# wienkers/marEx

Hardware: AMD Instinct MI355X
Metric: Mcells*timesteps/s, shifting_baseline + hobday_extreme p95 (validation+anomaly+thresholds+mask) (higher is better)
Workload: dtype f32

## Files before the change

### marex_amd/csrc/build.py

```python
import os
import subprocess
import sys
from concurrent.futures import ThreadPoolExecutor

HERE = os.path.dirname(os.path.abspath(__file__))
ROOT = os.path.dirname(os.path.dirname(HERE))
UNITS = ["marex_context", "marex_synth", "marex_shifting", "marex_thresholds", "marex_mask", "marex_anomalies",
         "marex_quantiles", "marex_morphology", "marex_objects", "marex_mesh_objects", "marex_merge", "marex_blosc", "marex_tails", "marex_zstd"]
SRC = [os.path.join(HERE, u + ".hip") for u in UNITS]
HEADERS = [os.path.join(HERE, "marex_common.hip.h"), os.path.join(HERE, "marex_tails.hip.h"), os.path.join(ROOT, "include", "marex_hip.h")]
OUT = os.path.join(HERE, "libmarex_hip.so")
FLAGS = [
    "--offload-arch=gfx950", "-O3", "-std=c++17", "-fPIC",
    "-ffp-contract=off",
    "-fno-fast-math", "-Wall", "-Wno-unused-result", "-Wno-unused-function",
    "-I", os.path.join(ROOT, "include"),
]


def _obj(src: str) -> str:
    return src[:-4] + ".o"


def _stale(target: str, deps) -> bool:
    if not os.path.exists(target):
        return True
    t = os.path.getmtime(target)
    return any(os.path.getmtime(d) > t for d in deps)


def needs_build() -> bool:
    return _stale(OUT, SRC + HEADERS + [os.path.abspath(__file__)])


def build(force: bool = False, verbose: bool = True) -> str:
    hipcc = os.environ.get("HIPCC", "/opt/rocm/bin/hipcc")
    extra = os.environ.get("MAREX_HIPCC_FLAGS", "").split()
    todo = [s for s in SRC if force or extra or _stale(_obj(s), [s] + HEADERS + [os.path.abspath(__file__)])]

    def compile_one(src):
        cmd = [hipcc, *FLAGS, *extra, "-c", src, "-o", _obj(src)]
        if verbose:
            print(" ".join(cmd), flush=True)
# ... 16 lines not shown
```

### marex_amd/csrc/marex_common.hip.h

```cpp
#pragma once
#include <hip/hip_runtime.h>

#include <cmath>
#include <type_traits>
#include <cstdarg>
#include <cstdio>
#include <cstring>
#include <map>
#include <string>
#include <vector>

#include "marex_hip.h"

#define NDOY MAREX_NDOY

struct TimedLaunch {
    int kid;
    hipEvent_t a, b;
};

struct marex_ctx {
    int device = 0;
    hipStream_t stream = nullptr;
    std::string err;
    bool timing = false;
    std::vector<TimedLaunch> pending;
    double total_ms[MAREX_K_COUNT] = {0};
    int64_t launches[MAREX_K_COUNT] = {0};
    int* shift_info = nullptr;
    int* shift_plan = nullptr;
    size_t shift_plan_years = 0;
    int* shift_lplan = nullptr;
    size_t shift_lplan_years = 0;
    unsigned char* thr_scratch = nullptr;
    size_t thr_scratch_bytes = 0;
    unsigned char* detrend_scratch = nullptr;
    size_t detrend_scratch_bytes = 0;
    unsigned char* morph_scratch = nullptr;
    size_t morph_scratch_bytes = 0;
    int n_cu = 0;
    std::map<std::string, int> opts;
    long long* row_off = nullptr;
    size_t row_off_bytes = 0;
    long long* row_off_mask = nullptr;
    size_t row_off_mask_bytes = 0;
    unsigned long long* dbg_counters = nullptr;
};

#define MAREX_DBG_COUNTERS 8

static inline int ctx_opt(marex_ctx* ctx, const char* name, int dflt) {
    auto it = ctx->opts.find(name);
    return it == ctx->opts.end() ? dflt : it->second;
}

#ifdef MAREX_ABLATION
#define MAREX_ABLATE_OPT(ctx, name) ctx_opt(ctx, name, 0)
#else
#define MAREX_ABLATE_OPT(ctx, name) 0
#endif

static inline unsigned long long* ctx_debug_counters(marex_ctx* ctx) {
    if (!ctx->dbg_counters) {
        if (hipMalloc((void**)&ctx->dbg_counters, MAREX_DBG_COUNTERS * sizeof(unsigned long long)) != hipSuccess) return nullptr;
        (void)hipMemsetAsync(ctx->dbg_counters, 0, MAREX_DBG_COUNTERS * sizeof(unsigned long long), ctx->stream);
    }
    return ctx->dbg_counters;
}
// ... 145 lines not shown
```

### marex_amd/csrc/marex_context.hip

```cpp
#include "marex_common.hip.h"

extern "C" int marex_abi_version(void) { return MAREX_ABI_VERSION; }

extern "C" int marex_workspace_bytes(const marex_workspace_cfg* cfg, size_t* bytes) {
    if (!cfg || !bytes || cfg->T <= 0 || cfg->T_out <= 0 || cfg->T_out > cfg->T || cfg->C <= 0) return -1;
    const size_t C = (size_t)cfg->C, To = (size_t)cfg->T_out;
    for (int i = 0; i < MAREX_WS_COUNT; ++i) bytes[i] = 0;
    bytes[MAREX_WS_ANOMALY] = To * C * sizeof(float);
    bytes[MAREX_WS_EXTREME] = To * C;
    bytes[MAREX_WS_THRESHOLDS] = (size_t)MAREX_NDOY * C * sizeof(float);
    if (cfg->list_rows > 0) {
        const int nper = marex_tail_lists(cfg->max_bucket, cfg->list_rows);
        if (nper < 1) return -1;
        const size_t nch = cfg->list_rows <= 16 ? 2 : 4;
        bytes[MAREX_WS_LISTS] = (size_t)MAREX_NDOY * (size_t)nper * nch * C * 16;
        bytes[MAREX_WS_AUX] = (size_t)MAREX_NDOY * C * sizeof(uint32_t);
    } else {
        bytes[MAREX_WS_BINS] = ((C + 15) / 16) * To * 16 * sizeof(uint16_t);
    }
    bytes[MAREX_WS_PER_CELL] = C * (sizeof(uint8_t) + sizeof(int32_t));
    bytes[MAREX_WS_TOTAL] = bytes[MAREX_WS_ANOMALY] + bytes[MAREX_WS_EXTREME] + 2 * bytes[MAREX_WS_THRESHOLDS] + bytes[MAREX_WS_LISTS] +
                            bytes[MAREX_WS_AUX] + bytes[MAREX_WS_BINS] + bytes[MAREX_WS_PER_CELL];
    return 0;
}
// ... 21 lines not shown
extern "C" int marex_set_option(marex_ctx* ctx, const char* name, int value) {
    if (!ctx || !name || !*name) return -1;
    ctx->opts[name] = value;
    return 0;
}

extern "C" int marex_clear_option(marex_ctx* ctx, const char* name) {
    if (!ctx) return -1;
    if (!name)
        ctx->opts.clear();
    else
        ctx->opts.erase(name);
    return 0;
}

extern "C" int marex_debug_counters(marex_ctx* ctx, uint64_t* out, int reset) {
    if (!ctx || !out) return -1;
    HIP_TRY(ctx, hipSetDevice(ctx->device));
    unsigned long long* d = ctx_debug_counters(ctx);
    if (!d) return fail(ctx, -2, "marex_debug_counters: allocation failed");
    HIP_TRY(ctx, hipStreamSynchronize(ctx->stream));
    HIP_TRY(ctx, hipMemcpy(out, d, MAREX_DBG_COUNTERS * sizeof(unsigned long long), hipMemcpyDeviceToHost));
    if (reset) HIP_TRY(ctx, hipMemsetAsync(d, 0, MAREX_DBG_COUNTERS * sizeof(unsigned long long), ctx->stream));
    return 0;
}

extern "C" int marex_destroy(marex_ctx* ctx) {
    if (!ctx) return -1;
    drain_timers(ctx);
    if (ctx->shift_info) (void)hipFree(ctx->shift_info);
    if (ctx->shift_plan) (void)hipFree(ctx->shift_plan);
    if (ctx->shift_lplan) (void)hipFree(ctx->shift_lplan);
    if (ctx->thr_scratch) (void)hipFree(ctx->thr_scratch);
    if (ctx->detrend_scratch) (void)hipFree(ctx->detrend_scratch);
    if (ctx->morph_scratch) (void)hipFree(ctx->morph_scratch);
    if (ctx->dbg_counters) (void)hipFree(ctx->dbg_counters);
    if (ctx->row_off) (void)hipFree(ctx->row_off);
    if (ctx->row_off_mask) (void)hipFree(ctx->row_off_mask);
    delete ctx;
    return 0;
}

extern "C" const char* marex_last_error(marex_ctx* ctx) { return ctx ? ctx->err.c_str() : "null context"; }

extern "C" int marex_set_stream(marex_ctx* ctx, void* s) {
    if (!ctx) return -1;
    ctx->stream = (hipStream_t)s;
    return 0;
}

extern "C" int marex_sync(marex_ctx* ctx) {
    if (!ctx) return -1;
    HIP_TRY(ctx, hipSetDevice(ctx->device));
    HIP_TRY(ctx, hipStreamSynchronize(ctx->stream));
    drain_timers(ctx);
    return 0;
}

extern "C" int marex_timing_enable(marex_ctx* ctx, int on) {
    if (!ctx) return -1;
    ctx->timing = on != 0;
    return 0;
}

extern "C" int marex_timing_reset(marex_ctx* ctx) {
    if (!ctx) return -1;
// ... 14 lines not shown
```

### marex_amd/csrc/marex_tails.hip

```cpp
#include "marex_common.hip.h"
#include "marex_tails.hip.h"

typedef __amdgpu_buffer_rsrc_t tl_rsrc_t;
__device__ __forceinline__ tl_rsrc_t tl_make_rsrc(const void* base) {
    return __builtin_amdgcn_make_buffer_rsrc(const_cast<void*>(base), 0, -1, 0x00020000);
}
__device__ __forceinline__ uint4 tl_load_chunk(tl_rsrc_t r, unsigned voff, unsigned soff) {
    typedef unsigned u4 __attribute__((ext_vector_type(4)));
    const u4 v = __builtin_amdgcn_raw_buffer_load_b128(r, (int)voff, (int)soff, 0);
    return make_uint4(v.x, v.y, v.z, v.w);
}
__device__ __forceinline__ unsigned pk_sub_sat_u16(unsigned a, unsigned b) {
    unsigned r;
    asm("v_pk_sub_u16 %0, %1, %2 clamp" : "=v"(r) : "v"(a), "v"(b));
    return r;
}
__device__ __forceinline__ unsigned pk_add_u16(unsigned a, unsigned b) {
    unsigned r;
    asm("v_pk_add_u16 %0, %1, %2" : "=v"(r) : "v"(a), "v"(b));
    return r;
}
__device__ __forceinline__ unsigned pk_sub_u16(unsigned a, unsigned b) {
    unsigned r;
    asm("v_pk_sub_u16 %0, %1, %2" : "=v"(r) : "v"(a), "v"(b));
    return r;
}
__device__ __forceinline__ unsigned pk_min1_u16(unsigned a) {
    unsigned r;
    asm("v_pk_min_u16 %0, %1, %2" : "=v"(r) : "v"(a), "v"(0x00010001u));
    return r;
}
__device__ __forceinline__ int tl_count_above(const uint4& ch, unsigned lim_rep) {
    const unsigned m0 = pk_min1_u16(pk_sub_sat_u16(ch.x, lim_rep)), m1 = pk_min1_u16(pk_sub_sat_u16(ch.y, lim_rep));
    const unsigned m2 = pk_min1_u16(pk_sub_sat_u16(ch.z, lim_rep)), m3 = pk_min1_u16(pk_sub_sat_u16(ch.w, lim_rep));
// ... 228 lines not shown
                     : [t] "=&v"(t), [a] "=&v"(a), [sv] "=&s"(sv)
                     : [n] "v"(n), [x] "v"(ch.x), [y] "v"(ch.y), [z] "v"(ch.z), [w] "v"(ch.w), [b0] "s"(B0), [hi] "s"(BWp1), [col] "v"(col_lds), [mul] "s"(mul)
                     : "vcc", "memory");
    else
        asm volatile(MAREX_BUMP_ALL("-1")
                     : [t] "=&v"(t), [a] "=&v"(a), [sv] "=&s"(sv)
                     : [n] "v"(n), [x] "v"(ch.x), [y] "v"(ch.y), [z] "v"(ch.z), [w] "v"(ch.w), [b0] "s"(B0), [hi] "s"(BWp1), [col] "v"(col_lds), [mul] "s"(mul)
                     : "vcc", "memory");
#undef MAREX_BUMP_ALL
#undef MAREX_BUMP_ADD
}
#undef MAREX_BUMP_KEY
#undef MAREX_BUMP_LO
#undef MAREX_BUMP_HI

#define TT_LS 34
#ifndef TT_BW
#define TT_BW 64
#endif
#define TT_MARGIN 6
#ifndef TT_STEP
#define TT_STEP 56
#endif
static_assert(TT_STEP <= TT_BW - 8, "straggler passes must overlap: a quantile bin between two tried bands would never be found");
#define TT_NPF 2

template <int NPERT>
struct TailBucket {
    uint4 c0[NPERT < TT_NPF ? NPERT : TT_NPF];
    unsigned aux;
    int d;
};

template <int P, int TC, int NT, int NPERT, int TR_ = NT / TC>
__global__ void __launch_bounds__(NT, NT == 256 ? 4 : (NT == 512 ? 2 : 1))
k_thr_tails(const uint4* __restrict__ lists, const unsigned* __restrict__ aux, int NPER, int nch, const float* __restrict__ anom,
            long C, int ny, int nx, int row0, int row1, int tiles_x, int Dd, const float* __restrict__ centres, int nb, double q,
            int wd, float lower_bound, float upper_bound, float* __restrict__ thr, marex_thr_stats* __restrict__ stats,
            unsigned long long* __restrict__ dbg, int pass_limit) {
    constexpr int TR = TR_;
    constexpr int NCELL = TR * TC;
    constexpr int NPF = NPERT < TT_NPF ? NPERT : TT_NPF;
    static_assert(NCELL <= NT && NT - NCELL < 64, "tile does not match the thread count");
    constexpr int OR = TR - 2 * P, OC = TC - 2 * P;
    __shared__ unsigned lev[NT * TT_LS];
    __shared__ unsigned tot_s[NT];
    __shared__ int s_lo[2], s_hi[2];
    __shared__ int s_iumin[2], s_iumax[2];
    __shared__ int s_est_min, s_est_max;

    const int t = threadIdx.x;
    const bool spare = NCELL < NT && t >= NCELL;
    const int tc = t % TC;
    const int tr = (TR > 1) ? (t / TC + P) % TR : 0;
    const int ci = spare ? t : tr * TC + tc;
    const int ty = (int)blockIdx.x / tiles_x, tx = (int)blockIdx.x - ty * tiles_x;
    const int jt0 = row0 + ty * OR, it0 = tx * OC;
    const int j = (ny > 0) ? jt0 - P + tr : 0;
    const int icol = it0 - P + tc;
    bool cell_valid;
    long cell;
    if (ny > 0) {
        int gi = icol % nx;
        if (gi < 0) gi += nx;
        cell_valid = (j >= 0 && j < ny) && !spare;
        cell = (long)j * nx + gi;
    } else {
        cell_valid = icol < nx && !spare;
        cell = icol < nx ? icol : nx - 1;
    }
    if (!cell_valid) cell = 0;
    const bool is_out = !spare && tr >= P && tr < TR - P && tc >= P && tc < TC - P && j < row1 && icol < nx && (ny > 0 ? j >= row0 : true);
    const int d_begin = (int)blockIdx.y * Dd;
    const int ndays = (NDOY - d_begin) < Dd ? (NDOY - d_begin) : Dd;
    const int pd = wd / 2;
    bool land = true;
    if (is_out) land = !(anom[cell] == anom[cell]);
    if (!__syncthreads_or(is_out && !land)) {
        if (is_out)
            for (int dd = 0; dd < ndays; ++dd) thr[(size_t)(d_begin + dd) * C + cell] = nan_f();
        return;
    }
    if (is_out && land)
        for (int dd = 0; dd < ndays; ++dd) thr[(size_t)(d_begin + dd) * C + cell] = nan_f();

    unsigned* mycol = &lev[ci * TT_LS];
    uint2* mycol2 = reinterpret_cast<uint2*>(mycol);
    typedef __attribute__((address_space(3))) unsigned lds_u32;
    const unsigned col_lds = (unsigned)(size_t)(lds_u32*)mycol;
    const int base_max = nb - TT_BW > 0 ? nb - TT_BW : 0;
    auto clamp_base = [&](int b) { return b < 0 ? 0 : (b > base_max ? base_max : b); };
    int B0 = 0;
    int BW = nb < TT_BW ? nb : TT_BW;
    constexpr int NLP = (TT_BW + 2 + 1) / 2;
    const unsigned voff = (unsigned)cell * 16u;
    const unsigned chunk_row = (unsigned)C * 16u;
    const size_t day_stride = (size_t)NPER * nch * (size_t)C;

    auto load_bucket = [&](int d0) {
        TailBucket<NPERT> b;
        b.d = d0;
        const tl_rsrc_t r = tl_make_rsrc(lists + (size_t)d0 * day_stride);
#pragma unroll
        for (int p = 0; p < NPF; ++p)
            b.c0[p] = (p < NPER) ? tl_load_chunk(r, voff, (unsigned)(nch * p) * chunk_row) : make_uint4(0, 0, 0, 0);
        b.aux = aux[(size_t)d0 * C + cell];
        return b;
    };
    auto bump = [&](int k, int sgn) {
        const int odd = k & 1;
        unsigned addr;
        asm("v_lshl_add_u32 %0, %1, 1, %2" : "=v"(addr) : "v"(k - odd), "v"(col_lds));
        int v;
        const int mul = sgn > 0 ? 65535 : -65535, one = sgn > 0 ? 1 : -1;
        asm("v_mad_i32_i24 %0, %1, %2, %3" : "=v"(v) : "v"(odd), "v"(mul), "v"(one));
        __hip_atomic_fetch_add((lds_u32*)(size_t)addr, (unsigned)v, __ATOMIC_RELAXED, __HIP_MEMORY_SCOPE_WORKGROUP);
    };
    int mytot = 0;
    constexpr bool ctx_asm_bump = true;
    auto bump_chunk = [&](const uint4& ch, int n, int sgn, int nfix) {
#pragma unroll
        for (int u = 0; u < 8; ++u) {
            const bool on = n > u;
            if (u >= nfix && __builtin_amdgcn_ballot_w64(on) == 0) break;
            if (on) {
                int lvl = tl_bin1(ch, u) - B0;
                lvl = lvl > BW + 1 ? BW + 1 : lvl;
                bump(lvl, sgn);
// ... 150 lines not shown
                continue;
            }
            cb = 0;
#pragma unroll
            for (int i = 0; i < 8; ++i) {
                if (i == n - 1) cb = Wv[i];
                if (i == n) ck = Wv[i];
            }
            return start + n;
        }
    };
    unsigned kmin = 0xFFFFFFFFu, kmax = 0u, nlow = 0u, nhigh = 0u;
    auto emit_threshold = [&](int d, int iu, int ck, int cb, double qpos) {
        const int il = iu > 0 ? iu - 1 : 0;
        const int cs_iu = ck;
        const int cs_il = iu > 0 ? cb : ck;
        const int diff = cs_iu - cs_il;
        const double frac = diff > 0 ? (qpos - (double)cs_il) / (double)diff : 0.5;
        const float dc = centres[iu] - centres[il];
        const double prod = frac * (double)dc;
        float t32 = (float)((double)centres[il] + prod);
        if (iu == 0) t32 = centres[0];
        const unsigned key = ordered_key(t32);
        kmin = key < kmin ? key : kmin;
        kmax = key > kmax ? key : kmax;
        if (t32 > upper_bound) ++nhigh;
        if (t32 < lower_bound) {
            ++nlow;
            t32 = lower_bound;
        }
        thr[(size_t)d * C + cell] = t32;
    };

    if (t == 0) {
        s_est_min = 0x7fffffff;
        s_est_max = -1;
        s_lo[0] = s_lo[1] = s_hi[0] = s_hi[1] = 0;
        s_iumin[0] = s_iumin[1] = 0x7fffffff;
        s_iumax[0] = s_iumax[1] = -1;
    }
    __syncthreads();
    {
        const TailBucket<NPERT> b = load_bucket(d_begin);
        const int cnt = cell_valid ? (int)(b.aux & 0x3FFu) : 0;
        if (cnt > 0) {
            int rank = (int)ceil((1.0 - q) * (double)cnt / (double)NPER);
            rank = rank < 1 ? 1 : (rank > 8 ? 8 : rank);
            unsigned key = 0;
#pragma unroll
            for (int u = 0; u < 8; ++u)
                if (u == rank - 1) key = tl_key(b.c0[0], u);
            if (key != 0u) {
                const int est = (int)(key >> TAIL_POS_BITS) - 1;
                atomicMin(&s_est_min, est);
                atomicMax(&s_est_max, est);
            }
        }
    }
    __syncthreads();
    {
        const int emin = s_est_min, emax = s_est_max;
        if (emax >= 0) {
            const int span = emax - emin + 1;
            B0 = clamp_base(span <= TT_BW - 2 * TT_MARGIN ? emin - (TT_BW - span) / 2 : emin - TT_MARGIN);
        }
    }
    BW = nb - B0 < TT_BW ? nb - B0 : TT_BW;

    int hint = -1;
    bool need_rebuild = true;
    unsigned long long n_rebuild = 0, n_pass = 0;
    TailBucket<NPERT> pin, pout;
    pin.d = pout.d = 0;
    pin.aux = pout.aux = 0;
#pragma unroll
    for (int p = 0; p < NPF; ++p) pin.c0[p] = pout.c0[p] = make_uint4(0, 0, 0, 0);
#ifdef MAREX_STAMPS
    unsigned long long st_p1 = 0, st_p2 = 0, st_bar = 0;
#define STAMP() __builtin_amdgcn_s_memtime()
#endif
    for (int dd = 0; dd < ndays; ++dd) {
        const int d = d_begin + dd;
        const int dpar = dd & 1;
#ifdef MAREX_STAMPS
        const unsigned long long tA = STAMP();
#endif
        if (need_rebuild) {
            rebuild(d);
            need_rebuild = false;
            ++n_rebuild;
            hint = -1;
        } else {
            unprefix();
            apply_bucket(pin, +1);
            apply_bucket(pout, -1);
        }
        tot_s[ci] = prefix();
        if (dd + 1 < ndays) {
            pin = load_bucket(wrap(d + 1 + pd));
            pout = load_bucket(wrap(d - pd));
        }
#ifdef MAREX_STAMPS
        const unsigned long long tB = STAMP();
        st_p1 += tB - tA;
#endif
        bool resolved = !(is_out && !land);
        int tried_lo = B0, tried_hi = B0;
        bool excursion = false;
        for (int pass = 0;; ++pass) {
            const int par = pass & 1;
#ifdef MAREX_STAMPS
            const unsigned long long tC0 = STAMP();
#endif
            __syncthreads();
#ifdef MAREX_STAMPS
            const unsigned long long tC = STAMP();
            st_bar += tC - tC0;
#endif
            if (t == 0) {
                s_lo[par ^ 1] = 0;
                s_hi[par ^ 1] = 0;
                if (pass == 0) {
                    s_iumin[dpar ^ 1] = 0x7fffffff;
                    s_iumax[dpar ^ 1] = -1;
                }
            }
            int iu_lo = 0x7fffffff, iu_hi = -1;
            if (!resolved) {
                const int tot = pooled_tot();
                if (tot > 0) {
                    const double qpos = q * (double)tot;
                    int ck, cb;
                    int k = find_level(hint, BW + 1, qpos, ck, cb);
                    int iu = -1;
                    if (k >= 1 && k <= BW) {
                        iu = B0 + k - 1;
                        hint = k;
                    } else if (k > BW && B0 + BW >= nb) {
                        iu = nb - 1;
                        k = iu - B0 + 1;
                        ck = pooled(k);
                        cb = pooled(k - 1);
                        hint = k;
                    } else if (k > BW) {
                        atomicOr(&s_hi[par], 1);
                        hint = -1;
                    } else {
                        atomicOr(&s_lo[par], 1);
                        hint = -1;
                    }
                    if (iu >= 0) {
                        emit_threshold(d, iu, ck, cb, qpos);
                        iu_lo = iu_hi = iu;
                        resolved = true;
                    }
                } else {
                    thr[(size_t)d * C + cell] = nan_f();
                    resolved = true;
                }
            }
            if (__builtin_amdgcn_ballot_w64(iu_hi >= 0) != 0) {
                const int wlo = wave_min_i32(iu_lo), whi = wave_max_i32(iu_hi);
                if ((t & 63) == 0) {
                    atomicMin(&s_iumin[dpar], wlo);
                    atomicMax(&s_iumax[dpar], whi);
                }
            }
#ifdef MAREX_STAMPS
            const unsigned long long tD = STAMP();
            st_p2 += tD - tC;
#endif
            __syncthreads();
#ifdef MAREX_STAMPS
            st_bar += STAMP() - tD;
#endif
            const int lo = s_lo[par], hi = s_hi[par];
            if (!lo && !hi) break;
            if (pass >= pass_limit) {
                if (!resolved) {
                    thr[(size_t)d * C + cell] = nan_f();
                    atomicAdd(&stats->n_unresolved, 1u);
                }
                break;
            }
            if (lo) {
                B0 = clamp_base(tried_lo - TT_STEP);
                tried_lo = B0;
            } else {
                B0 = clamp_base(tried_hi + TT_STEP);
                tried_hi = B0;
            }
            BW = nb - B0 < TT_BW ? nb - B0 : TT_BW;
            excursion = true;
            rebuild(d);
            tot_s[ci] = prefix();
            hint = -1;
            ++n_pass;
        }
        if (dd + 1 < ndays) {
            const int imin = s_iumin[dpar], imax = s_iumax[dpar];
            if (imax >= 0) {
                const int span = imax - imin + 1;
                const bool near_edge = imin - B0 < TT_MARGIN || (B0 + BW - 1) - imax < TT_MARGIN;
                if (excursion || near_edge) {
                    const int want = clamp_base(span <= TT_BW - 2 * TT_MARGIN ? imin - (TT_BW - span) / 2 : imin - TT_MARGIN);
                    if (want != B0) {
                        B0 = want;
                        BW = nb - B0 < TT_BW ? nb - B0 : TT_BW;
                        need_rebuild = true;
                    }
                }
            }
        }
    }
    for (int sft = 32; sft > 0; sft >>= 1) {
        const unsigned a = __shfl_down(kmin, sft, 64), b = __shfl_down(kmax, sft, 64);
        kmin = a < kmin ? a : kmin;
        kmax = b > kmax ? b : kmax;
        nlow += __shfl_down(nlow, sft, 64);
        nhigh += __shfl_down(nhigh, sft, 64);
    }
    if ((t & 63) == 0) {
        if (kmin != 0xFFFFFFFFu) atomicMin(&stats->min_key, kmin);
        if (kmax != 0u) atomicMax(&stats->max_key, kmax);
        if (nlow) atomicAdd(&stats->n_too_low, nlow);
        if (nhigh) atomicAdd(&stats->n_too_high, nhigh);
    }
#ifdef MAREX_STAMPS
#ifdef MAREX_STAMPS_WAVE
    const int st_wave = MAREX_STAMPS_WAVE >= 0 ? MAREX_STAMPS_WAVE : (int)((blockIdx.x + blockIdx.y) % (NT / 64));
    if (dbg && t == st_wave * 64) {
#else
    if (dbg && t == 0) {
#endif
        atomicAdd(&dbg[5], st_p1);
        atomicAdd(&dbg[6], st_p2);
        atomicAdd(&dbg[7], st_bar);
    }
#endif
    if (dbg && t == 0) {
        atomicAdd(&dbg[0], n_rebuild);
        atomicAdd(&dbg[2], n_pass);
        atomicAdd(&dbg[3], (unsigned long long)ndays);
    }
}

template <int NSC>
__global__ void __launch_bounds__(64)
k_thr_cells(const uint4* __restrict__ lists, const unsigned* __restrict__ aux, int NPER, int nch, const float* __restrict__ anom,
            long C, long c0, long c1, int nblk, const float* __restrict__ centres, int nb, double q, int wd, float lower_bound,
            float upper_bound, float* __restrict__ thr, marex_thr_stats* __restrict__ stats, unsigned long long* __restrict__ dbg) {
    extern __shared__ uint4 ring[];
    const int lane = (int)threadIdx.x;
    const long cell_raw = c0 + (long)blockIdx.x * 64 + lane;
    const bool valid = cell_raw < c1;
    const long cell = valid ? cell_raw : c1 - 1;
    const int d_begin = (int)blockIdx.y * NDOY / nblk, d_end = ((int)blockIdx.y + 1) * NDOY / nblk;
    const bool land = !(anom[cell] == anom[cell]);
    if (__builtin_amdgcn_ballot_w64(valid && !land) == 0) {
        if (valid)
            for (int d = d_begin; d < d_end; ++d) thr[(size_t)d * C + cell] = nan_f();
        return;
    }
    const int pd = wd / 2, nslot = (wd * NPER + 3) & ~3;
    uint4* mine = ring + lane;
    for (int k = wd * NPER; k < nslot; ++k) mine[k * 64] = make_uint4(0, 0, 0, 0);
    const unsigned voff = (unsigned)cell * 16u, chunk_row = (unsigned)C * 16u;
    const size_t day_stride = (size_t)NPER * nch * (size_t)C;
    auto wrap = [](int d) { return d < 0 ? d + NDOY : (d >= NDOY ? d - NDOY : d); };
    auto cnt_of = [&](int day) { return (int)(aux[(size_t)day * C + cell] & 0x3FFu); };
    auto load_day = [&](int day, int k) {
        const tl_rsrc_t r = tl_make_rsrc(lists + (size_t)day * day_stride);
        for (int p = 0; p < NPER; ++p) mine[((k % wd) * NPER + p) * 64] = tl_load_chunk(r, voff, (unsigned)(nch * p) * chunk_row);
    };
    int tot = 0;
    for (int o = 0; o < wd; ++o) {
// ... 185 lines not shown
        int nblk = (int)((32L * 4 * device_cus(ctx) + ncg - 1) / ncg);
        nblk = nblk < 1 ? 1 : (nblk > 12 ? 12 : nblk);
        nblk = ctx_opt(ctx, "THR_CELLS_BLOCKS", nblk);
        LaunchTimer lt(ctx, MAREX_K_THRESHOLDS);
        const size_t lds = (size_t)((wd * NPER + 3) & ~3) * 64 * sizeof(uint4);
        const int nslot = (wd * NPER + 3) & ~3;
        const bool cached = nslot == 12 && ctx_opt(ctx, "THR_CELLS_CACHE", 1);
        if (lds > 64 * 1024) HIP_TRY(ctx, hipFuncSetAttribute((const void*)k_thr_cells<0>, hipFuncAttributeMaxDynamicSharedMemorySize, (int)lds));
        hipLaunchKernelGGL(cached ? k_thr_cells<12> : k_thr_cells<0>, dim3((unsigned)ncg, (unsigned)nblk), dim3(64), lds, ctx->stream,
                           reinterpret_cast<const uint4*>(lists), aux, NPER, nch, anom, (long)C, c0, c1, nblk, centres, nb, q, wd,
                           lower_bound, upper_bound, thr_doy_major, stats, ctx_debug_counters(ctx));
        HIP_TRY(ctx, hipGetLastError());
        return 0;
    }
    if (NPER > 6)
        return fail(ctx, -4, "marex_hobday_thresholds_tails_f32: %d rows per bucket in lists of %d: more than 6 lists", max_bucket, list_rows);
    const int tile_pref = ctx_opt(ctx, "THR_TILE", (ny > 0 && p > 0 && max_bucket >= 24) ? 32 : 16);
    const bool half = (ny > 0 && p == 2) && tile_pref == 3216 && (row1 - row0) >= 12 && nx >= 16;
    const bool big = !half && (ny > 0 && p > 0) && tile_pref == 32 && (row1 - row0) >= 16 && nx >= 16;
    const int NT = big ? 1024 : (half ? 512 : 256);
    int TR = (ny > 0 && p > 0) ? (big ? 32 : 16) : 1, TC = NT / TR;
    const size_t lds_pad = (size_t)ctx_opt(ctx, "THR_LDS_PAD", 0) * 1024;
    bool tall = false;
    if (big && p == 2 && ctx_opt(ctx, "THR_TALL", 1)) {
        auto ntiles = [&](int tr, int tc) {
            return (long)((nx + tc - 2 * p - 1) / (tc - 2 * p)) * ((row1 - row0 + tr - 2 * p - 1) / (tr - 2 * p));
        };
        tall = ntiles(34, 30) < ntiles(32, 32) && (row1 - row0) >= 30;
        if (tall) TR = 34, TC = 30;
    }
    const int OR = TR - 2 * p, OC = TC - 2 * p;
    const int tiles_x = (nx + OC - 1) / OC, tiles_y = (row1 - row0 + OR - 1) / OR;
    int Dd = ctx_opt(ctx, "THR_DD", 0);
    if (Dd < 1 || Dd > NDOY) {
        const long cus = device_cus(ctx), tiles = (long)tiles_x * tiles_y;
        const long slots = cus * (big ? 1 : (half ? 2 : 4));
        long best = -1;
        for (int d = 16; d <= NDOY; ++d) {
            const long blocks = tiles * ((NDOY + d - 1) / d);
            const long cost = ((blocks + slots - 1) / slots) * (d + wd);
            if (best < 0 || cost < best) best = cost, Dd = d;
        }
    }
    dim3 grid((unsigned)(tiles_x * tiles_y), (unsigned)((NDOY + Dd - 1) / Dd));
    unsigned long long* dbg = ctx_debug_counters(ctx);
    const uint4* tl = reinterpret_cast<const uint4*>(lists);
    const int pass_limit = ctx_opt(ctx, "THR_PASS_LIMIT", 2 * (nb / TT_STEP) + 9);
#define MAREX_TT_ARGS tl, aux, NPER, nch, anom, (long)C, ny, nx, row0, row1, tiles_x, Dd, centres, nb, q, wd, lower_bound, upper_bound, thr_doy_major, stats, dbg, pass_limit
#define MAREX_TT_LAUNCH(PP, TCC, NTT, ...)                                                                                           \
    do {                                                                                                                             \
        if (NPER <= 1)                                                                                                               \
            hipLaunchKernelGGL((k_thr_tails<PP, TCC, NTT, 1, ##__VA_ARGS__>), grid, dim3(NTT), lds_pad, ctx->stream, MAREX_TT_ARGS); \
        else if (NPER <= 2)                                                                                                          \
            hipLaunchKernelGGL((k_thr_tails<PP, TCC, NTT, 2, ##__VA_ARGS__>), grid, dim3(NTT), lds_pad, ctx->stream, MAREX_TT_ARGS); \
        else                                                  \
            hipLaunchKernelGGL((k_thr_tails<PP, TCC, NTT, 3, ##__VA_ARGS__>), grid, dim3(NTT), lds_pad, ctx->stream, MAREX_TT_ARGS); \
    } while (0)
    {
        LaunchTimer lt(ctx, MAREX_K_THRESHOLDS);
        if (TR == 1)
            MAREX_TT_LAUNCH(0, 256, 256);
        else if (half)
            MAREX_TT_LAUNCH(2, 32, 512, 16);
        else if (big && p == 1)
            MAREX_TT_LAUNCH(1, 32, 1024);
        else if (big && p == 2 && tall)
            MAREX_TT_LAUNCH(2, 30, 1024, 34);
        else if (big && p == 2)
            MAREX_TT_LAUNCH(2, 32, 1024);
        else if (big)
            MAREX_TT_LAUNCH(3, 32, 1024);
        else if (p == 1)
            MAREX_TT_LAUNCH(1, 16, 256);
        else if (p == 2)
            MAREX_TT_LAUNCH(2, 16, 256);
        else
            MAREX_TT_LAUNCH(3, 16, 256);
    }
#undef MAREX_TT_LAUNCH
#undef MAREX_TT_ARGS
    HIP_TRY(ctx, hipGetLastError());
    return 0;
}
// ... 263 lines not shown
```

Baseline: 323,200.

## Compact live threshold tiles and balance day ranges across a persistent grid

Land-only tiles are now classified and NaN-filled by a separate pre-pass kernel, and a single-block compaction kernel builds a list of live tiles. The tails kernel then runs as a persistent grid sized to device slots. Each workgroup walks a contiguous range of (live tile, day) positions, with cut points adjusted to avoid tiny segments near year boundaries. The intent is to remove the load imbalance and idle blocks caused by mostly-land tiles in the fixed tiles×day-chunk grid. In exchange it adds two extra launches, a serial compaction step and per-segment re-setup overhead inside the kernel.

Result: slower. 319,800 (-1.1%).

```diff
diff --git a/marex_amd/csrc/build.py b/marex_amd/csrc/build.py
--- a/marex_amd/csrc/build.py
+++ b/marex_amd/csrc/build.py
@@ -8,7 +8,8 @@
 UNITS = ["marex_context", "marex_synth", "marex_shifting", "marex_thresholds", "marex_mask", "marex_anomalies",
          "marex_quantiles", "marex_morphology", "marex_objects", "marex_mesh_objects", "marex_merge", "marex_blosc", "marex_tails", "marex_zstd"]
 SRC = [os.path.join(HERE, u + ".hip") for u in UNITS]
-HEADERS = [os.path.join(HERE, "marex_common.hip.h"), os.path.join(HERE, "marex_tails.hip.h"), os.path.join(ROOT, "include", "marex_hip.h")]
+HEADERS = [os.path.join(HERE, "marex_common.hip.h"), os.path.join(HERE, "marex_tails.hip.h"), os.path.join(HERE, "marex_thr_walk.h"),
+           os.path.join(ROOT, "include", "marex_hip.h")]
 OUT = os.path.join(HERE, "libmarex_hip.so")
 FLAGS = [
     "--offload-arch=gfx950", "-O3", "-std=c++17", "-fPIC",
diff --git a/marex_amd/csrc/marex_common.hip.h b/marex_amd/csrc/marex_common.hip.h
--- a/marex_amd/csrc/marex_common.hip.h
+++ b/marex_amd/csrc/marex_common.hip.h
@@ -34,6 +34,8 @@
     size_t shift_lplan_years = 0;
     unsigned char* thr_scratch = nullptr;
     size_t thr_scratch_bytes = 0;
+    int* thr_walk = nullptr;
+    size_t thr_walk_ints = 0;
     unsigned char* detrend_scratch = nullptr;
     size_t detrend_scratch_bytes = 0;
     unsigned char* morph_scratch = nullptr;
diff --git a/marex_amd/csrc/marex_context.hip b/marex_amd/csrc/marex_context.hip
--- a/marex_amd/csrc/marex_context.hip
+++ b/marex_amd/csrc/marex_context.hip
@@ -77,6 +77,7 @@
     if (ctx->shift_plan) (void)hipFree(ctx->shift_plan);
     if (ctx->shift_lplan) (void)hipFree(ctx->shift_lplan);
     if (ctx->thr_scratch) (void)hipFree(ctx->thr_scratch);
+    if (ctx->thr_walk) (void)hipFree(ctx->thr_walk);
     if (ctx->detrend_scratch) (void)hipFree(ctx->detrend_scratch);
     if (ctx->morph_scratch) (void)hipFree(ctx->morph_scratch);
     if (ctx->dbg_counters) (void)hipFree(ctx->dbg_counters);
diff --git a/marex_amd/csrc/marex_tails.hip b/marex_amd/csrc/marex_tails.hip
--- a/marex_amd/csrc/marex_tails.hip
+++ b/marex_amd/csrc/marex_tails.hip
@@ -1,5 +1,6 @@
 #include "marex_common.hip.h"
 #include "marex_tails.hip.h"
+#include "marex_thr_walk.h"
 
 typedef __amdgpu_buffer_rsrc_t tl_rsrc_t;
 __device__ __forceinline__ tl_rsrc_t tl_make_rsrc(const void* base) {
@@ -294,57 +295,114 @@
     int d;
 };
 
+struct TileLane {
+    long cell;
+    bool cell_valid;
+    bool is_out;
+};
+template <int P, int TC, int NT, int TR>
+__device__ __forceinline__ TileLane tt_tile_lane(int tile, int t, int ny, int nx, int row0, int row1, int tiles_x) {
+    constexpr int NCELL = TR * TC;
+    constexpr int OR = TR - 2 * P, OC = TC - 2 * P;
+    const bool spare = NCELL < NT && t >= NCELL;
+    const int tc = t % TC;
+    const int tr = (TR > 1) ? (t / TC + P) % TR : 0;
+    const int ty = tile / tiles_x, tx = tile - ty * tiles_x;
+    const int jt0 = row0 + ty * OR, it0 = tx * OC;
+    const int j = (ny > 0) ? jt0 - P + tr : 0;
+    const int icol = it0 - P + tc;
+    TileLane L;
+    if (ny > 0) {
+        int gi = icol % nx;
+        if (gi < 0) gi += nx;
+        L.cell_valid = (j >= 0 && j < ny) && !spare;
+        L.cell = (long)j * nx + gi;
+    } else {
+        L.cell_valid = icol < nx && !spare;
+        L.cell = icol < nx ? icol : nx - 1;
+    }
+    if (!L.cell_valid) L.cell = 0;
+    L.is_out = !spare && tr >= P && tr < TR - P && tc >= P && tc < TC - P && j < row1 && icol < nx && (ny > 0 ? j >= row0 : true);
+    return L;
+}
+__device__ __forceinline__ bool tt_lane_land(const TileLane& L, const float* __restrict__ anom) {
+    return L.is_out ? !(anom[L.cell] == anom[L.cell]) : true;
+}
+
+template <int P, int TC, int NT, int TR_ = NT / TC>
+__global__ void __launch_bounds__(NT)
+k_thr_tiles(const float* __restrict__ anom, long C, int ny, int nx, int row0, int row1, int tiles_x, float* __restrict__ thr,
+            int* __restrict__ flag) {
+    const TileLane L = tt_tile_lane<P, TC, NT, TR_>((int)blockIdx.x, (int)threadIdx.x, ny, nx, row0, row1, tiles_x);
+    const bool live = __syncthreads_or(L.is_out && !tt_lane_land(L, anom)) != 0;
+    if (threadIdx.x == 0) flag[blockIdx.x] = live ? 1 : 0;
+    if (!live && L.is_out)
+        for (int d = 0; d < NDOY; ++d) thr[(size_t)d * C + L.cell] = nan_f();
+}
+
+__global__ void __launch_bounds__(1024)
+k_thr_compact(const int* __restrict__ flag, int ntiles, int* __restrict__ walk) {
+    __shared__ int s_wave[16];
+    __shared__ int s_base;
+    const int t = threadIdx.x, wv = t >> 6, ln = t & 63;
+    if (t == 0) s_base = 0;
+    __syncthreads();
+    for (int b = 0; b < ntiles; b += 1024) {
+        const int i = b + t;
+        const bool on = i < ntiles && flag[i] != 0;
+        const unsigned long long m = __builtin_amdgcn_ballot_w64(on);
+        if (ln == 0) s_wave[wv] = __popcll(m);
+        __syncthreads();
+        int before = s_base;
+        for (int k = 0; k < wv; ++k) before += s_wave[k];
+        if (on) walk[1 + before + __popcll(m & ((1ull << ln) - 1ull))] = i;
+        __syncthreads();
+        if (t == 1023) s_base = before + s_wave[15];
+        __syncthreads();
+    }
+    if (t == 0) walk[0] = s_base;
+}
+
+#define TT_WALKS(P) ((P) < 3)
+
 template <int P, int TC, int NT, int NPERT, int TR_ = NT / TC>
 __global__ void __launch_bounds__(NT, NT == 256 ? 4 : (NT == 512 ? 2 : 1))
 k_thr_tails(const uint4* __restrict__ lists, const unsigned* __restrict__ aux, int NPER, int nch, const float* __restrict__ anom,
-            long C, int ny, int nx, int row0, int row1, int tiles_x, int Dd, const float* __restrict__ centres, int nb, double q,
+            long C, int ny, int nx, int row0, int row1, int tiles_x, int Dd, const int* __restrict__ walk,
+            const float* __restrict__ centres, int nb, double q,
             int wd, float lower_bound, float upper_bound, float* __restrict__ thr, marex_thr_stats* __restrict__ stats,
             unsigned long long* __restrict__ dbg, int pass_limit) {
     constexpr int TR = TR_;
+    constexpr bool WALK = TT_WALKS(P);
     constexpr int NCELL = TR * TC;
     constexpr int NPF = NPERT < TT_NPF ? NPERT : TT_NPF;
     static_assert(NCELL <= NT && NT - NCELL < 64, "tile does not match the thread count");
-    constexpr int OR = TR - 2 * P, OC = TC - 2 * P;
     __shared__ unsigned lev[NT * TT_LS];
     __shared__ unsigned tot_s[NT];
     __shared__ int s_lo[2], s_hi[2];
     __shared__ int s_iumin[2], s_iumax[2];
     __shared__ int s_est_min, s_est_max;
+    __shared__ int s_alive;
 
     const int t = threadIdx.x;
     const bool spare = NCELL < NT && t >= NCELL;
     const int tc = t % TC;
     const int tr = (TR > 1) ? (t / TC + P) % TR : 0;
     const int ci = spare ? t : tr * TC + tc;
-    const int ty = (int)blockIdx.x / tiles_x, tx = (int)blockIdx.x - ty * tiles_x;
-    const int jt0 = row0 + ty * OR, it0 = tx * OC;
-    const int j = (ny > 0) ? jt0 - P + tr : 0;
-    const int icol = it0 - P + tc;
-    bool cell_valid;
-    long cell;
-    if (ny > 0) {
-        int gi = icol % nx;
-        if (gi < 0) gi += nx;
-        cell_valid = (j >= 0 && j < ny) && !spare;
-        cell = (long)j * nx + gi;
+    int pos, pos_end;
+    if (Dd > 0) {
+        const int d0 = (int)blockIdx.y * Dd;
+        pos = (int)blockIdx.x * NDOY + d0;
+        pos_end = pos + ((NDOY - d0) < Dd ? (NDOY - d0) : Dd);
     } else {
-        cell_valid = icol < nx && !spare;
-        cell = icol < nx ? icol : nx - 1;
-    }
-    if (!cell_valid) cell = 0;
-    const bool is_out = !spare && tr >= P && tr < TR - P && tc >= P && tc < TC - P && j < row1 && icol < nx && (ny > 0 ? j >= row0 : true);
-    const int d_begin = (int)blockIdx.y * Dd;
-    const int ndays = (NDOY - d_begin) < Dd ? (NDOY - d_begin) : Dd;
+        const marex_thr_range r = marex_thr_walk_range(walk[0], gridDim.x, 4 * wd, wd, blockIdx.x);
+        pos = __builtin_amdgcn_readfirstlane((int)r.begin);
+        pos_end = __builtin_amdgcn_readfirstlane((int)r.end);
+    }
     const int pd = wd / 2;
-    bool land = true;
-    if (is_out) land = !(anom[cell] == anom[cell]);
-    if (!__syncthreads_or(is_out && !land)) {
-        if (is_out)
-            for (int dd = 0; dd < ndays; ++dd) thr[(size_t)(d_begin + dd) * C + cell] = nan_f();
-        return;
-    }
-    if (is_out && land)
-        for (int dd = 0; dd < ndays; ++dd) thr[(size_t)(d_begin + dd) * C + cell] = nan_f();
+    bool cell_valid = false, is_out = false, land = true;
+    long cell = 0;
+    unsigned voff = 0;
 
     unsigned* mycol = &lev[ci * TT_LS];
     uint2* mycol2 = reinterpret_cast<uint2*>(mycol);
@@ -355,7 +413,6 @@
     int B0 = 0;
     int BW = nb < TT_BW ? nb : TT_BW;
     constexpr int NLP = (TT_BW + 2 + 1) / 2;
-    const unsigned voff = (unsigned)cell * 16u;
     const unsigned chunk_row = (unsigned)C * 16u;
     const size_t day_stride = (size_t)NPER * nch * (size_t)C;
 
@@ -572,187 +629,215 @@
         thr[(size_t)d * C + cell] = t32;
     };
 
-    if (t == 0) {
-        s_est_min = 0x7fffffff;
-        s_est_max = -1;
-        s_lo[0] = s_lo[1] = s_hi[0] = s_hi[1] = 0;
-        s_iumin[0] = s_iumin[1] = 0x7fffffff;
-        s_iumax[0] = s_iumax[1] = -1;
-    }
-    __syncthreads();
-    {
-        const TailBucket<NPERT> b = load_bucket(d_begin);
-        const int cnt = cell_valid ? (int)(b.aux & 0x3FFu) : 0;
-        if (cnt > 0) {
-            int rank = (int)ceil((1.0 - q) * (double)cnt / (double)NPER);
-            rank = rank < 1 ? 1 : (rank > 8 ? 8 : rank);
-            unsigned key = 0;
-#pragma unroll
-            for (int u = 0; u < 8; ++u)
-                if (u == rank - 1) key = tl_key(b.c0[0], u);
-            if (key != 0u) {
-                const int est = (int)(key >> TAIL_POS_BITS) - 1;
-                atomicMin(&s_est_min, est);
-                atomicMax(&s_est_max, est);
-            }
-        }
-    }
-    __syncthreads();
-    {
-        const int emin = s_est_min, emax = s_est_max;
-        if (emax >= 0) {
-            const int span = emax - emin + 1;
-            B0 = clamp_base(span <= TT_BW - 2 * TT_MARGIN ? emin - (TT_BW - span) / 2 : emin - TT_MARGIN);
-        }
-    }
-    BW = nb - B0 < TT_BW ? nb - B0 : TT_BW;
-
-    int hint = -1;
-    bool need_rebuild = true;
-    unsigned long long n_rebuild = 0, n_pass = 0;
-    TailBucket<NPERT> pin, pout;
-    pin.d = pout.d = 0;
-    pin.aux = pout.aux = 0;
-#pragma unroll
-    for (int p = 0; p < NPF; ++p) pin.c0[p] = pout.c0[p] = make_uint4(0, 0, 0, 0);
+    unsigned long long n_rebuild = 0, n_pass = 0, n_days = 0;
 #ifdef MAREX_STAMPS
     unsigned long long st_p1 = 0, st_p2 = 0, st_bar = 0;
 #define STAMP() __builtin_amdgcn_s_memtime()
 #endif
-    for (int dd = 0; dd < ndays; ++dd) {
-        const int d = d_begin + dd;
-        const int dpar = dd & 1;
+    TailBucket<NPERT> pin, pout;
+    pin.d = pout.d = 0;
+    pin.aux = pout.aux = 0;
+#pragma unroll
+    for (int p = 0; p < NPF; ++p) pin.c0[p] = pout.c0[p] = make_uint4(0, 0, 0, 0);
+    if (pos < pos_end) do {
+        const int ti = pos / NDOY, d_begin = pos - ti * NDOY;
+        const int ndays = (NDOY - d_begin) < (pos_end - pos) ? (NDOY - d_begin) : (pos_end - pos);
+        const int tile = Dd > 0 ? ti : walk[1 + ti];
+        pos += ndays;
+        {
+            int t_seg = t;
+            asm volatile("" : "+v"(t_seg));
+            const TileLane L = tt_tile_lane<P, TC, NT, TR>(tile, t_seg, ny, nx, row0, row1, tiles_x);
+            cell = L.cell;
+            cell_valid = L.cell_valid;
+            is_out = L.is_out;
+            land = tt_lane_land(L, anom);
+            voff = (unsigned)cell * 16u;
+        }
+        if (is_out && land)
+            for (int dd = 0; dd < ndays; ++dd) thr[(size_t)(d_begin + dd) * C + cell] = nan_f();
+        __syncthreads();
+        if (t == 0) {
+            int z = 0;
+            asm volatile("" : "+v"(z));
+            s_alive = z;
+            s_est_min = z ^ 0x7fffffff;
+            s_est_max = ~z;
+            s_lo[0] = s_lo[1] = s_hi[0] = s_hi[1] = z;
+            s_iumin[0] = s_iumin[1] = z ^ 0x7fffffff;
+            s_iumax[0] = s_iumax[1] = ~z;
+        }
+        B0 = 0;
+        __syncthreads();
+        if (is_out && !land) s_alive = 1;
+        {
+            const TailBucket<NPERT> b = load_bucket(d_begin);
+            const int cnt = cell_valid ? (int)(b.aux & 0x3FFu) : 0;
+            if (cnt > 0) {
+                double q_seg = q;
+                asm volatile("" : "+s"(q_seg));
+                int rank = (int)ceil((1.0 - q_seg) * (double)cnt / (double)NPER);
+                rank = rank < 1 ? 1 : (rank > 8 ? 8 : rank);
+                unsigned key = 0;
+#pragma unroll
+                for (int u = 0; u < 8; ++u)
+                    if (u == rank - 1) key = tl_key(b.c0[0], u);
+                if (key != 0u) {
+                    const int est = (int)(key >> TAIL_POS_BITS) - 1;
+                    atomicMin(&s_est_min, est);
+                    atomicMax(&s_est_max, est);
+                }
+            }
+        }
+        __syncthreads();
+        if (!s_alive) continue;
+        {
+            const int emin = s_est_min, emax = s_est_max;
+            if (emax >= 0) {
+                const int span = emax - emin + 1;
+                B0 = clamp_base(span <= TT_BW - 2 * TT_MARGIN ? emin - (TT_BW - span) / 2 : emin - TT_MARGIN);
+            }
+        }
+        BW = nb - B0 < TT_BW ? nb - B0 : TT_BW;
+
+        int hint = -1;
+        bool need_rebuild = true;
+        for (int dd = 0; dd < ndays; ++dd) {
+            const int d = d_begin + dd;
+            const int dpar = dd & 1;
 #ifdef MAREX_STAMPS
-        const unsigned long long tA = STAMP();
+            const unsigned long long tA = STAMP();
 #endif
-        if (need_rebuild) {
-            rebuild(d);
-            need_rebuild = false;
-            ++n_rebuild;
-            hint = -1;
-        } else {
-            unprefix();
-            apply_bucket(pin, +1);
-            apply_bucket(pout, -1);
-        }
-        tot_s[ci] = prefix();
-        if (dd + 1 < ndays) {
-            pin = load_bucket(wrap(d + 1 + pd));
-            pout = load_bucket(wrap(d - pd));
-        }
+            if (need_rebuild) {
+                rebuild(d);
+                need_rebuild = false;
+                ++n_rebuild;
+                hint = -1;
+            } else {
+                unprefix();
+                apply_bucket(pin, +1);
+                apply_bucket(pout, -1);
+            }
+            tot_s[ci] = prefix();
+            if (dd + 1 < ndays) {
+                pin = load_bucket(wrap(d + 1 + pd));
+                pout = load_bucket(wrap(d - pd));
+            }
 #ifdef MAREX_STAMPS
-        const unsigned long long tB = STAMP();
-        st_p1 += tB - tA;
+            const unsigned long long tB = STAMP();
+            st_p1 += tB - tA;
 #endif
-        bool resolved = !(is_out && !land);
-        int tried_lo = B0, tried_hi = B0;
-        bool excursion = false;
-        for (int pass = 0;; ++pass) {
-            const int par = pass & 1;
+            bool resolved = !(is_out && !land);
+            int tried_lo = B0, tried_hi = B0;
+            bool excursion = false;
+            for (int pass = 0;; ++pass) {
+                const int par = pass & 1;
 #ifdef MAREX_STAMPS
-            const unsigned long long tC0 = STAMP();
+                const unsigned long long tC0 = STAMP();
 #endif
-            __syncthreads();
+                __syncthreads();
 #ifdef MAREX_STAMPS
-            const unsigned long long tC = STAMP();
-            st_bar += tC - tC0;
+                const unsigned long long tC = STAMP();
+                st_bar += tC - tC0;
 #endif
-            if (t == 0) {
-                s_lo[par ^ 1] = 0;
-                s_hi[par ^ 1] = 0;
-                if (pass == 0) {
-                    s_iumin[dpar ^ 1] = 0x7fffffff;
-                    s_iumax[dpar ^ 1] = -1;
-                }
-            }
-            int iu_lo = 0x7fffffff, iu_hi = -1;
-            if (!resolved) {
-                const int tot = pooled_tot();
-                if (tot > 0) {
-                    const double qpos = q * (double)tot;
-                    int ck, cb;
-                    int k = find_level(hint, BW + 1, qpos, ck, cb);
-                    int iu = -1;
-                    if (k >= 1 && k <= BW) {
-                        iu = B0 + k - 1;
-                        hint = k;
-                    } else if (k > BW && B0 + BW >= nb) {
-                        iu = nb - 1;
-                        k = iu - B0 + 1;
-                        ck = pooled(k);
-                        cb = pooled(k - 1);
-                        hint = k;
-                    } else if (k > BW) {
-                        atomicOr(&s_hi[par], 1);
-                        hint = -1;
+                if (t == 0) {
+                    s_lo[par ^ 1] = 0;
+                    s_hi[par ^ 1] = 0;
+                    if (pass == 0) {
+                        s_iumin[dpar ^ 1] = 0x7fffffff;
+                        s_iumax[dpar ^ 1] = -1;
+                    }
+                }
+                int iu_lo = 0x7fffffff, iu_hi = -1;
+                if (!resolved) {
+                    const int tot = pooled_tot();
+                    if (tot > 0) {
+                        const double qpos = q * (double)tot;
+                        int ck, cb;
+                        int k = find_level(hint, BW + 1, qpos, ck, cb);
+                        int iu = -1;
+                        if (k >= 1 && k <= BW) {
+                            iu = B0 + k - 1;
+                            hint = k;
+                        } else if (k > BW && B0 + BW >= nb) {
+                            iu = nb - 1;
+                            k = iu - B0 + 1;
+                            ck = pooled(k);
+                            cb = pooled(k - 1);
+                            hint = k;
+                        } else if (k > BW) {
+                            atomicOr(&s_hi[par], 1);
+                            hint = -1;
+                        } else {
+                            atomicOr(&s_lo[par], 1);
+                            hint = -1;
+                        }
+                        if (iu >= 0) {
+                            emit_threshold(d, iu, ck, cb, qpos);
+                            iu_lo = iu_hi = iu;
+                            resolved = true;
+                        }
                     } else {
-                        atomicOr(&s_lo[par], 1);
-                        hint = -1;
-                    }
-                    if (iu >= 0) {
-                        emit_threshold(d, iu, ck, cb, qpos);
-                        iu_lo = iu_hi = iu;
+                        thr[(size_t)d * C + cell] = nan_f();
                         resolved = true;
                     }
+                }
+                if (__builtin_amdgcn_ballot_w64(iu_hi >= 0) != 0) {
+                    const int wlo = wave_min_i32(iu_lo), whi = wave_max_i32(iu_hi);
+                    if ((t & 63) == 0) {
+                        atomicMin(&s_iumin[dpar], wlo);
+                        atomicMax(&s_iumax[dpar], whi);
+                    }
+                }
+#ifdef MAREX_STAMPS
+                const unsigned long long tD = STAMP();
+                st_p2 += tD - tC;
+#endif
+                __syncthreads();
+#ifdef MAREX_STAMPS
+                st_bar += STAMP() - tD;
+#endif
+                const int lo = s_lo[par], hi = s_hi[par];
+                if (!lo && !hi) break;
+                if (pass >= pass_limit) {
+                    if (!resolved) {
+                        thr[(size_t)d * C + cell] = nan_f();
+                        atomicAdd(&stats->n_unresolved, 1u);
+                    }
+                    break;
+                }
+                if (lo) {
+                    B0 = clamp_base(tried_lo - TT_STEP);
+                    tried_lo = B0;
                 } else {
-                    thr[(size_t)d * C + cell] = nan_f();
-                    resolved = true;
-                }
-            }
-            if (__builtin_amdgcn_ballot_w64(iu_hi >= 0) != 0) {
-                const int wlo = wave_min_i32(iu_lo), whi = wave_max_i32(iu_hi);
-                if ((t & 63) == 0) {
-                    atomicMin(&s_iumin[dpar], wlo);
-                    atomicMax(&s_iumax[dpar], whi);
-                }
-            }
-#ifdef MAREX_STAMPS
-            const unsigned long long tD = STAMP();
-            st_p2 += tD - tC;
-#endif
-            __syncthreads();
-#ifdef MAREX_STAMPS
-            st_bar += STAMP() - tD;
-#endif
-            const int lo = s_lo[par], hi = s_hi[par];
-            if (!lo && !hi) break;
-            if (pass >= pass_limit) {
-                if (!resolved) {
-                    thr[(size_t)d * C + cell] = nan_f();
-                    atomicAdd(&stats->n_unresolved, 1u);
-                }
-                break;
-            }
-            if (lo) {
-                B0 = clamp_base(tried_lo - TT_STEP);
-                tried_lo = B0;
-            } else {
-                B0 = clamp_base(tried_hi + TT_STEP);
-                tried_hi = B0;
-            }
-            BW = nb - B0 < TT_BW ? nb - B0 : TT_BW;
-            excursion = true;
-            rebuild(d);
-            tot_s[ci] = prefix();
-            hint = -1;
-            ++n_pass;
-        }
-        if (dd + 1 < ndays) {
-            const int imin = s_iumin[dpar], imax = s_iumax[dpar];
-            if (imax >= 0) {
-                const int span = imax - imin + 1;
-                const bool near_edge = imin - B0 < TT_MARGIN || (B0 + BW - 1) - imax < TT_MARGIN;
-                if (excursion || near_edge) {
-                    const int want = clamp_base(span <= TT_BW - 2 * TT_MARGIN ? imin - (TT_BW - span) / 2 : imin - TT_MARGIN);
-                    if (want != B0) {
-                        B0 = want;
-                        BW = nb - B0 < TT_BW ? nb - B0 : TT_BW;
-                        need_rebuild = true;
+                    B0 = clamp_base(tried_hi + TT_STEP);
+                    tried_hi = B0;
+                }
+                BW = nb - B0 < TT_BW ? nb - B0 : TT_BW;
+                excursion = true;
+                rebuild(d);
+                tot_s[ci] = prefix();
+                hint = -1;
+                ++n_pass;
+            }
+            if (dd + 1 < ndays) {
+                const int imin = s_iumin[dpar], imax = s_iumax[dpar];
+                if (imax >= 0) {
+                    const int span = imax - imin + 1;
+                    const bool near_edge = imin - B0 < TT_MARGIN || (B0 + BW - 1) - imax < TT_MARGIN;
+                    if (excursion || near_edge) {
+                        const int want = clamp_base(span <= TT_BW - 2 * TT_MARGIN ? imin - (TT_BW - span) / 2 : imin - TT_MARGIN);
+                        if (want != B0) {
+                            B0 = want;
+                            BW = nb - B0 < TT_BW ? nb - B0 : TT_BW;
+                            need_rebuild = true;
+                        }
                     }
                 }
             }
         }
-    }
+        n_days += (unsigned long long)ndays;
+    } while (WALK && pos < pos_end);
     for (int sft = 32; sft > 0; sft >>= 1) {
         const unsigned a = __shfl_down(kmin, sft, 64), b = __shfl_down(kmax, sft, 64);
         kmin = a < kmin ? a : kmin;
@@ -778,10 +863,10 @@
         atomicAdd(&dbg[7], st_bar);
     }
 #endif
-    if (dbg && t == 0) {
+    if (dbg && t == 0 && n_days) {
         atomicAdd(&dbg[0], n_rebuild);
         atomicAdd(&dbg[2], n_pass);
-        atomicAdd(&dbg[3], (unsigned long long)ndays);
+        atomicAdd(&dbg[3], n_days);
     }
 }
 
@@ -1033,9 +1118,10 @@
     const int OR = TR - 2 * p, OC = TC - 2 * p;
     const int tiles_x = (nx + OC - 1) / OC, tiles_y = (row1 - row0 + OR - 1) / OR;
     int Dd = ctx_opt(ctx, "THR_DD", 0);
-    if (Dd < 1 || Dd > NDOY) {
-        const long cus = device_cus(ctx), tiles = (long)tiles_x * tiles_y;
-        const long slots = cus * (big ? 1 : (half ? 2 : 4));
+    if (Dd < 1 || Dd > NDOY) Dd = 0;
+    const long tiles = (long)tiles_x * tiles_y;
+    const long slots = (long)device_cus(ctx) * (big ? 1 : (half ? 2 : 4));
+    if (!Dd && !TT_WALKS(p)) {
         long best = -1;
         for (int d = 16; d <= NDOY; ++d) {
             const long blocks = tiles * ((NDOY + d - 1) / d);
@@ -1043,13 +1129,30 @@
             if (best < 0 || cost < best) best = cost, Dd = d;
         }
     }
-    dim3 grid((unsigned)(tiles_x * tiles_y), (unsigned)((NDOY + Dd - 1) / Dd));
+    long G = ctx_opt(ctx, "THR_WGS", (int)slots);
+    G = G < 1 ? 1 : (G > (1L << 20) ? (1L << 20) : G);
+    const size_t walk_ints = 1 + 2 * (size_t)tiles;
+    if (ctx->thr_walk_ints < walk_ints) {
+        if (ctx->thr_walk) {
+            HIP_TRY(ctx, hipFree(ctx->thr_walk));
+            ctx->thr_walk = nullptr;
+            ctx->thr_walk_ints = 0;
+        }
+        HIP_TRY(ctx, hipMalloc((void**)&ctx->thr_walk, walk_ints * sizeof(int)));
+        ctx->thr_walk_ints = walk_ints;
+    }
+    int* const walk = ctx->thr_walk;
+    int* const flag = walk + 1 + tiles;
+    const dim3 grid = Dd ? dim3((unsigned)tiles, (unsigned)((NDOY + Dd - 1) / Dd)) : dim3((unsigned)G);
     unsigned long long* dbg = ctx_debug_counters(ctx);
     const uint4* tl = reinterpret_cast<const uint4*>(lists);
     const int pass_limit = ctx_opt(ctx, "THR_PASS_LIMIT", 2 * (nb / TT_STEP) + 9);
-#define MAREX_TT_ARGS tl, aux, NPER, nch, anom, (long)C, ny, nx, row0, row1, tiles_x, Dd, centres, nb, q, wd, lower_bound, upper_bound, thr_doy_major, stats, dbg, pass_limit
+#define MAREX_TT_ARGS tl, aux, NPER, nch, anom, (long)C, ny, nx, row0, row1, tiles_x, Dd, walk, centres, nb, q, wd, lower_bound, upper_bound, thr_doy_major, stats, dbg, pass_limit
 #define MAREX_TT_LAUNCH(PP, TCC, NTT, ...)                                                                                           \
     do {                                                                                                                             \
+        hipLaunchKernelGGL((k_thr_tiles<PP, TCC, NTT, ##__VA_ARGS__>), dim3((unsigned)tiles), dim3(NTT), 0, ctx->stream, anom,       \
+                           (long)C, ny, nx, row0, row1, tiles_x, thr_doy_major, flag);                                               \
+        if (!Dd) hipLaunchKernelGGL(k_thr_compact, dim3(1), dim3(1024), 0, ctx->stream, flag, (int)tiles, walk);                     \
         if (NPER <= 1)                                                                                                               \
             hipLaunchKernelGGL((k_thr_tails<PP, TCC, NTT, 1, ##__VA_ARGS__>), grid, dim3(NTT), lds_pad, ctx->stream, MAREX_TT_ARGS); \
         else if (NPER <= 2)                                                                                                          \
diff --git a/marex_amd/csrc/marex_thr_walk.h b/marex_amd/csrc/marex_thr_walk.h
--- /dev/null
+++ b/marex_amd/csrc/marex_thr_walk.h
@@ -0,0 +1,37 @@
+#pragma once
+#if defined(__HIPCC__)
+#define MAREX_WALK_HD __host__ __device__
+#else
+#define MAREX_WALK_HD
+#endif
+
+#define MAREX_WALK_DAYS 366
+
+struct marex_thr_range {
+    long long begin, end;
+};
+
+MAREX_WALK_HD inline long long marex_thr_walk_len(long long n_live, long long n_wg, long long q_min) {
+    const long long total = n_live * MAREX_WALK_DAYS;
+    long long q = n_wg > 0 ? (total + n_wg - 1) / n_wg : total;
+    if (q < q_min) q = q_min;
+    return q < 1 ? 1 : q;
+}
+
+MAREX_WALK_HD inline long long marex_thr_walk_cut(long long p, long long total, int m) {
+    if (p <= 0) return 0;
+    if (p >= total) return total;
+    if (m > MAREX_WALK_DAYS / 3) m = MAREX_WALK_DAYS / 3;
+    const long long r = p % MAREX_WALK_DAYS, s = MAREX_WALK_DAYS - r, t0 = p - r;
+    if (r < m) return 2 * r <= m ? t0 : t0 + m;
+    if (s < m) return 2 * s <= m ? t0 + MAREX_WALK_DAYS : t0 + MAREX_WALK_DAYS - m;
+    return p;
+}
+
+MAREX_WALK_HD inline marex_thr_range marex_thr_walk_range(long long n_live, long long n_wg, long long q_min, int m, long long w) {
+    const long long total = n_live * MAREX_WALK_DAYS, q = marex_thr_walk_len(n_live, n_wg, q_min);
+    marex_thr_range r;
+    r.begin = marex_thr_walk_cut(w * q < total ? w * q : total, total, m);
+    r.end = marex_thr_walk_cut((w + 1) * q < total ? (w + 1) * q : total, total, m);
+    return r;
+}
```
